# zhaozijie2022/LocoTouch

Hardware: AMD Instinct MI355X
Metric: env-steps/sec (whole node), TransportTeacher 4096 envs/GPU (higher is better)
Workload: dtype f32

## Files before the change

locotouch_amd/csrc/lt_wgrad.hip:

```cpp
#include <hip/hip_runtime.h>
#include <stdint.h>

#include "lt_env.h"
#include "lt_host_check.h"
#include "lt_internal.h"

namespace {

typedef float f32x4 __attribute__((ext_vector_type(4)));
typedef float f32x2 __attribute__((ext_vector_type(2)));
typedef _Float16 f16x8 __attribute__((ext_vector_type(8)));
typedef _Float16 f16x2 __attribute__((ext_vector_type(2)));

constexpr int TA = 4, TB = 4;
constexpr float LO_SCALE = 64.f;

template <int U>
__device__ __forceinline__ void split8(const f32x4 (&v)[8], float scale, f16x8& hi, f16x8& lo) {
#pragma unroll
  for (int p = 0; p < 4; ++p) {
    f32x2 x;
    x[0] = v[2 * p][U] * scale; x[1] = v[2 * p + 1][U] * scale;
    const f16x2 h = __builtin_convertvector(x, f16x2);
    const f32x2 d = (x - __builtin_convertvector(h, f32x2)) * LO_SCALE;
    const f16x2 l = __builtin_convertvector(d, f16x2);
    hi[2 * p] = h[0]; hi[2 * p + 1] = h[1];
    lo[2 * p] = l[0]; lo[2 * p + 1] = l[1];
  }
}

template <int U>
__device__ __forceinline__ void unpack8(const f32x4 (&v)[8], f16x8& hi, f16x8& lo) {
  typedef unsigned u32x4 __attribute__((ext_vector_type(4)));
  u32x4 h, l;
#pragma unroll
  for (int p = 0; p < 4; ++p) {
    const unsigned w0 = __float_as_uint(v[2 * p][U]), w1 = __float_as_uint(v[2 * p + 1][U]);
    h[p] = __builtin_amdgcn_perm(w1, w0, 0x05040100u);
    l[p] = __builtin_amdgcn_perm(w1, w0, 0x07060302u);
  }
  hi = __builtin_bit_cast(f16x8, h);
  lo = __builtin_bit_cast(f16x8, l);
}

struct WgradArgs {
  const float* dz;
  const float* x;
  long long M;
  int N, K;
  int tiles_n, tiles_k, splits;
  const float* amax;
  int nblk_amax;
  float* slabs;
  int dz_split;
  const float* dz_scale;
  int x_split;
  float* db;
};

constexpr int WG_WAVES = 4;
template <bool AS, bool XS>
__global__ __launch_bounds__(64 * WG_WAVES, 2) void lt_wgrad_kernel(const WgradArgs a) {
  __shared__ f32x4 s_tile[WG_WAVES - 1][TA * TB + 1][64];
  const int lane = threadIdx.x & 63;
  const int wave = __builtin_amdgcn_readfirstlane((int)threadIdx.x >> 6);
  const int i = lane & 15, g = lane >> 4;
  const int tiles = a.tiles_n * a.tiles_k;
  const int per_xcd = (int)gridDim.x >> 3;
  const int item = ((int)blockIdx.x & 7) * per_xcd + ((int)blockIdx.x >> 3);
  if (item >= tiles * a.splits) return;
  const int split = item / tiles, tile = item - split * tiles;
  const int tn = tile / a.tiles_k, tk = tile - tn * a.tiles_k;
  const int n0 = tn * 16 * TA, k0 = tk * 16 * TB;
  const long long steps = (a.M + 31) / 32;
  const long long b0 = steps * split / a.splits, b1 = steps * (split + 1) / a.splits;
  const long long s0 = b0 + (b1 - b0) * wave / WG_WAVES, s1 = b0 + (b1 - b0) * (wave + 1) / WG_WAVES;
  float scale = 1.f;
  if (AS) {
    scale = *a.dz_scale;
  } else if (a.amax) {
    float m = 0.f;
    for (int b = lane; b < a.nblk_amax; b += 64) m = fmaxf(m, a.amax[b]);
#pragma unroll
    for (int off = 32; off > 0; off >>= 1) m = fmaxf(m, __shfl_xor(m, off, 64));
    const int e = (int)((__float_as_uint(m) >> 23) & 0xFF) - 127;
    int se = 7 - e;
    se = se > 100 ? 100 : (se < -100 ? -100 : se);
    scale = __uint_as_float((unsigned)(127 + se) << 23);
  }
  f32x4 acc[TA][TB];
#pragma unroll
  for (int p = 0; p < TA; ++p)
#pragma unroll
    for (int q = 0; q < TB; ++q) acc[p][q] = f32x4{0.f, 0.f, 0.f, 0.f};
  f32x4 va[8], vb[8];
  const int ca = min(n0 + 4 * i, a.N - 4), cb = min(k0 + 4 * i, a.K - 4);
  const unsigned row_a = (unsigned)a.N * 4u, row_b = (unsigned)a.K * 4u;
  const unsigned last_a = (unsigned)(a.M - 1) * row_a + (unsigned)ca * 4u, last_b = (unsigned)(a.M - 1) * row_b + (unsigned)cb * 4u;
  unsigned off_a = ((unsigned)s0 * 32u + (unsigned)g) * row_a + (unsigned)ca * 4u, off_b = ((unsigned)s0 * 32u + (unsigned)g) * row_b + (unsigned)cb * 4u;
  auto issue = [&](long long) __attribute__((always_inline)) {
#pragma unroll
    for (int t = 0; t < 8; ++t) {
      va[t] = *(const f32x4*)((const char*)a.dz + min(off_a + (unsigned)(4 * t) * row_a, last_a));
      vb[t] = *(const f32x4*)((const char*)a.x + min(off_b + (unsigned)(4 * t) * row_b, last_b));
    }
    off_a += 32u * row_a;
    off_b += 32u * row_b;
  };
  const bool colsum = a.db != nullptr && tk == 0;
  f32x4 cs = f32x4{0.f, 0.f, 0.f, 0.f};
  if (s0 < s1) issue(s0);
  for (long long s = s0; s < s1; ++s) {
    if ((s + 1) * 32 > a.M) {
#pragma unroll
      for (int t = 0; t < 8; ++t) if (s * 32 + 4 * t + g >= a.M) va[t] = f32x4{0.f, 0.f, 0.f, 0.f};
    }
    if (colsum) {
      if (AS) {
#pragma unroll
        for (int t = 0; t < 8; ++t)
#pragma unroll
          for (int u = 0; u < 4; ++u) {
            const unsigned w = __float_as_uint(va[t][u]);
            cs[u] += (float)__builtin_bit_cast(_Float16, (unsigned short)(w & 0xFFFFu)) + (float)__builtin_bit_cast(_Float16, (unsigned short)(w >> 16)) * (1.f / LO_SCALE);
          }
      } else {
#pragma unroll
        for (int t = 0; t < 8; ++t) cs += va[t];
      }
    }
    f16x8 ah[TA], al[TA], bh[TB], bl[TB];
    if (AS) {
      unpack8<0>(va, ah[0], al[0]); unpack8<1>(va, ah[1], al[1]); unpack8<2>(va, ah[2], al[2]); unpack8<3>(va, ah[3], al[3]);
    } else {
      split8<0>(va, scale, ah[0], al[0]); split8<1>(va, scale, ah[1], al[1]); split8<2>(va, scale, ah[2], al[2]); split8<3>(va, scale, ah[3], al[3]);
    }
    if (XS) {
      unpack8<0>(vb, bh[0], bl[0]); unpack8<1>(vb, bh[1], bl[1]); unpack8<2>(vb, bh[2], bl[2]); unpack8<3>(vb, bh[3], bl[3]);
    } else {
      split8<0>(vb, 1.f, bh[0], bl[0]); split8<1>(vb, 1.f, bh[1], bl[1]); split8<2>(vb, 1.f, bh[2], bl[2]); split8<3>(vb, 1.f, bh[3], bl[3]);
    }
    if (s + 1 < s1) issue(s + 1);
#pragma unroll
    for (int p = 0; p < TA; ++p) {
      const f16x8 a64 = ah[p] * (_Float16)LO_SCALE;
#pragma unroll
      for (int q = 0; q < TB; ++q) {
        acc[p][q] = __builtin_amdgcn_mfma_f32_16x16x32_f16(a64, bh[q], acc[p][q], 0, 0, 0);
        acc[p][q] = __builtin_amdgcn_mfma_f32_16x16x32_f16(ah[p], bl[q], acc[p][q], 0, 0, 0);
        acc[p][q] = __builtin_amdgcn_mfma_f32_16x16x32_f16(al[p], bh[q], acc[p][q], 0, 0, 0);
      }
    }
  }
  if (wave > 0) {
#pragma unroll
    for (int p = 0; p < TA; ++p)
#pragma unroll
      for (int q = 0; q < TB; ++q) s_tile[wave - 1][p * TB + q][lane] = acc[p][q];
    s_tile[wave - 1][TA * TB][lane] = cs;
  }
  __syncthreads();
  if (wave > 0) return;
#pragma unroll
  for (int w = 0; w < WG_WAVES - 1; ++w) {
#pragma unroll
    for (int p = 0; p < TA; ++p)
#pragma unroll
      for (int q = 0; q < TB; ++q) acc[p][q] += s_tile[w][p * TB + q][lane];
    cs += s_tile[w][TA * TB][lane];
  }
  if (colsum) {
#pragma unroll
    for (int u = 0; u < 4; ++u) {
      cs[u] += __shfl_xor(cs[u], 16, 64);
      cs[u] += __shfl_xor(cs[u], 32, 64);
    }
    if (AS) cs *= 1.f / scale;
    if (g == 0 && n0 + 4 * i < a.N) *(f32x4*)(a.db + (long long)split * a.N + n0 + 4 * i) = cs;
  }
  const float inv = 1.f / (scale * LO_SCALE);
  float* const out = a.slabs + (long long)split * a.N * a.K;
  const int k = k0 + 4 * i;
#pragma unroll
  for (int p = 0; p < TA; ++p)
#pragma unroll
    for (int r = 0; r < 4; ++r) {
      const int n = n0 + 4 * (4 * g + r) + p;
      if (n < a.N && k < a.K) {
        f32x4 o;
#pragma unroll
        for (int q = 0; q < TB; ++q) o[q] = acc[p][q][r] * inv;
        *(f32x4*)(out + (long long)n * a.K + k) = o;
      }
    }
}

int pick_splits(long long M, int tiles) {
  const long long steps = (M + 31) / 32;
  long long s = 512 / tiles;
  if (s > steps / 8) s = steps / 8;
  return (int)(s < 1 ? 1 : s);
}

}

extern "C" int lt_wgrad_splits(int64_t M, int N, int K) {
  const int tiles = ((N + 16 * TA - 1) / (16 * TA)) * ((K + 16 * TB - 1) / (16 * TB));
  return pick_splits((long long)M, tiles);
}

extern "C" int64_t lt_wgrad_ws_floats(int64_t M, int N, int K) { return (int64_t)lt_wgrad_splits(M, N, K) * N * K; }

extern "C" int lt_wgrad(const float* dz, int dz_split, const float* dz_scale, const float* x, int x_split, int64_t M, int N, int K, const float* amax_blocks,
                        int nblk_amax, float* slabs, float* db_slabs, void* stream) {
  if (!dz || !x || !slabs || M < 1 || N < 4 || K < 4 || (N & 3) || (K & 3) || (amax_blocks && nblk_amax < 1) || (long long)M * (N > K ? N : K) * 4 >= (1ll << 32))
    return einval("lt_wgrad: invalid argument (N and K multiples of 4, each operand below 4 GiB)");
  WgradArgs a;
  a.dz = dz; a.x = x; a.M = M; a.N = N; a.K = K;
  a.amax = amax_blocks; a.nblk_amax = amax_blocks ? nblk_amax : 0;
  a.slabs = slabs; a.db = db_slabs; a.x_split = x_split != 0; a.dz_split = dz_split != 0; a.dz_scale = dz_scale;
  if (a.dz_split && !dz_scale) return einval("lt_wgrad: a split dz needs its scale");
  a.tiles_n = (N + 16 * TA - 1) / (16 * TA);
  a.tiles_k = (K + 16 * TB - 1) / (16 * TB);
  a.splits = pick_splits((long long)M, a.tiles_n * a.tiles_k);
  const dim3 grid((unsigned)((a.tiles_n * a.tiles_k * a.splits + 7) / 8 * 8));
  if (a.dz_split && a.x_split) hipLaunchKernelGGL((lt_wgrad_kernel<true, true>), grid, dim3(64 * WG_WAVES), 0, (hipStream_t)stream, a);
  else if (a.x_split) hipLaunchKernelGGL((lt_wgrad_kernel<false, true>), grid, dim3(64 * WG_WAVES), 0, (hipStream_t)stream, a);
  else if (a.dz_split) hipLaunchKernelGGL((lt_wgrad_kernel<true, false>), grid, dim3(64 * WG_WAVES), 0, (hipStream_t)stream, a);
  else hipLaunchKernelGGL((lt_wgrad_kernel<false, false>), grid, dim3(64 * WG_WAVES), 0, (hipStream_t)stream, a);
  return launch_status();
}

namespace {
__global__ __launch_bounds__(256) void lt_split_rows_kernel(const float* __restrict__ x, unsigned* __restrict__ out, long long n4) {
  typedef unsigned u32x4 __attribute__((ext_vector_type(4)));
  const long long i = (long long)blockIdx.x * 256 + threadIdx.x;
  if (i >= n4) return;
  const f32x4 v = ((const f32x4*)x)[i];
  u32x4 o;
#pragma unroll
  for (int k = 0; k < 4; ++k) {
    const float c = __builtin_amdgcn_fmed3f(v[k], -(float)LT_MLP_INPUT_CLAMP, (float)LT_MLP_INPUT_CLAMP);
    const _Float16 h = (_Float16)c;
    const _Float16 l = (_Float16)((c - (float)h) * LO_SCALE);
    o[k] = (unsigned)__builtin_bit_cast(unsigned short, h) | ((unsigned)__builtin_bit_cast(unsigned short, l) << 16);
  }
  ((u32x4*)out)[i] = o;
}
}

extern "C" int lt_split_rows(const float* x, void* out, int64_t count, void* stream) {
  if (!x || !out || count < 4 || (count & 3)) return einval("lt_split_rows: invalid argument (count a multiple of 4)");
  hipLaunchKernelGGL(lt_split_rows_kernel, dim3((unsigned)((count / 4 + 255) / 256)), dim3(256), 0, (hipStream_t)stream, x, (unsigned*)out, (long long)(count / 4));
  return launch_status();
}
```

Measured before the change: 68.32 million.

## Share split operand fragments across waves via LDS in wgrad kernel

Restructures the weight-gradient kernel so each workgroup covers a 2x2 block of 64x64 tiles with eight waves in two quads. In each quad, a wave loads and splits only one operand (dz or x) and exchanges the fp16 hi/lo fragments with a neighbour through double-buffered LDS. This removes the duplicate global loads and split work that separate tiles did before. It adds an LDS barrier per step, dynamic LDS allocation, and different split/grid sizing (MAX_WG 256, steps/4).

```diff
diff --git a/locotouch_amd/csrc/lt_wgrad.hip b/locotouch_amd/csrc/lt_wgrad.hip
--- a/locotouch_amd/csrc/lt_wgrad.hip
+++ b/locotouch_amd/csrc/lt_wgrad.hip
@@ -48,7 +48,7 @@
   const float* x;
   long long M;
   int N, K;
-  int tiles_n, tiles_k, splits;
+  int blocks_n, blocks_k, splits;
   const float* amax;
   int nblk_amax;
   float* slabs;
@@ -58,23 +58,119 @@
   float* db;
 };
 
-constexpr int WG_WAVES = 4;
+template <bool SPLIT>
+__device__ __forceinline__ void fragments(const f32x4 (&v)[8], float scale, f16x8 (&hi)[4], f16x8 (&lo)[4]) {
+  if (SPLIT) {
+    unpack8<0>(v, hi[0], lo[0]); unpack8<1>(v, hi[1], lo[1]); unpack8<2>(v, hi[2], lo[2]); unpack8<3>(v, hi[3], lo[3]);
+  } else {
+    split8<0>(v, scale, hi[0], lo[0]); split8<1>(v, scale, hi[1], lo[1]); split8<2>(v, scale, hi[2], lo[2]); split8<3>(v, scale, hi[3], lo[3]);
+  }
+}
+
+__device__ __forceinline__ void mma_tile(f32x4 (&acc)[TA][TB], const f16x8 (&ah)[TA], const f16x8 (&al)[TA], const f16x8 (&bh)[TB], const f16x8 (&bl)[TB]) {
+#pragma unroll
+  for (int p = 0; p < TA; ++p) {
+    const f16x8 a64 = ah[p] * (_Float16)LO_SCALE;
+#pragma unroll
+    for (int q = 0; q < TB; ++q) {
+      acc[p][q] = __builtin_amdgcn_mfma_f32_16x16x32_f16(a64, bh[q], acc[p][q], 0, 0, 0);
+      acc[p][q] = __builtin_amdgcn_mfma_f32_16x16x32_f16(ah[p], bl[q], acc[p][q], 0, 0, 0);
+      acc[p][q] = __builtin_amdgcn_mfma_f32_16x16x32_f16(al[p], bh[q], acc[p][q], 0, 0, 0);
+    }
+  }
+}
+
+__device__ __forceinline__ void lds_barrier() { asm volatile("s_waitcnt lgkmcnt(0)\n\ts_barrier" ::: "memory"); }
+
+constexpr int QUAD = 4;
+constexpr int WG_WAVES = 2 * QUAD;
+constexpr int PF = 1;
+constexpr int PANEL = 8 * 64;
+constexpr int LDS_BYTES = 2 * 2 * QUAD * PANEL * 16;
+constexpr int MAX_WG = 256;
+
+template <bool OWN_A, bool SPLIT, bool AS, bool COLSUM>
+__device__ __forceinline__ void sweep(const char* base, int M, int width, int col0, int g, int h0, int m_end, int trips, float scale, f16x8* post,
+                                      const f16x8* take, f32x4 (&acc)[TA][TB], f32x4& cs) {
+  const int col = min(col0, width - 4);
+  const unsigned row = (unsigned)width * 4u;
+  const unsigned last = (unsigned)(M - 1) * row + (unsigned)col * 4u;
+  unsigned off = ((unsigned)h0 * 32u + (unsigned)g) * row + (unsigned)col * 4u;
+  auto issue = [&](f32x4 (&v)[8]) __attribute__((always_inline)) {
+#pragma unroll
+    for (int t = 0; t < 8; ++t) v[t] = *(const f32x4*)(base + min(off + (unsigned)(4 * t) * row, last));
+    off += 32u * row;
+  };
+  f32x4 raw[PF][8];
+#pragma unroll
+  for (int j = 0; j < PF; ++j) {
+    issue(raw[j]);
+    __builtin_amdgcn_sched_barrier(0);
+  }
+  for (int it = 0; it < trips; it += PF) {
+#pragma unroll
+    for (int j = 0; j < PF; ++j) {
+      f32x4 (&v)[8] = raw[j];
+      const int left = m_end - (h0 + it + j) * 32 - g;
+#pragma unroll
+      for (int t = 0; t < 8; ++t)
+#pragma unroll
+        for (int u = 0; u < 4; ++u) v[t][u] = 4 * t < left ? v[t][u] : 0.f;
+      if (COLSUM) {
+        if (AS) {
+#pragma unroll
+          for (int t = 0; t < 8; ++t)
+#pragma unroll
+            for (int u = 0; u < 4; ++u) {
+              const unsigned w = __float_as_uint(v[t][u]);
+              cs[u] += (float)__builtin_bit_cast(_Float16, (unsigned short)(w & 0xFFFFu)) + (float)__builtin_bit_cast(_Float16, (unsigned short)(w >> 16)) * (1.f / LO_SCALE);
+            }
+        } else {
+#pragma unroll
+          for (int t = 0; t < 8; ++t) cs += v[t];
+        }
+      }
+      f16x8 oh[4], ol[4], fh[4], fl[4];
+      fragments<SPLIT>(v, scale, oh, ol);
+      const int buf = ((it + j) & 1) * QUAD * PANEL;
+#pragma unroll
+      for (int u = 0; u < 4; ++u) {
+        post[buf + (2 * u) * 64] = oh[u];
+        post[buf + (2 * u + 1) * 64] = ol[u];
+      }
+      issue(v);
+      lds_barrier();
+#pragma unroll
+      for (int u = 0; u < 4; ++u) {
+        fh[u] = take[buf + (2 * u) * 64];
+        fl[u] = take[buf + (2 * u + 1) * 64];
+      }
+      if (OWN_A) mma_tile(acc, oh, ol, fh, fl);
+      else mma_tile(acc, fh, fl, oh, ol);
+    }
+  }
+}
+
 template <bool AS, bool XS>
-__global__ __launch_bounds__(64 * WG_WAVES, 2) void lt_wgrad_kernel(const WgradArgs a) {
-  __shared__ f32x4 s_tile[WG_WAVES - 1][TA * TB + 1][64];
+__global__ __launch_bounds__(64 * WG_WAVES) void lt_wgrad_kernel(const WgradArgs a) {
+  extern __shared__ __attribute__((aligned(16))) unsigned char s_lds[];
   const int lane = threadIdx.x & 63;
   const int wave = __builtin_amdgcn_readfirstlane((int)threadIdx.x >> 6);
+  const int quad = wave >> 2, wq = wave & 3;
   const int i = lane & 15, g = lane >> 4;
-  const int tiles = a.tiles_n * a.tiles_k;
+  const int blocks = a.blocks_n * a.blocks_k;
   const int per_xcd = (int)gridDim.x >> 3;
   const int item = ((int)blockIdx.x & 7) * per_xcd + ((int)blockIdx.x >> 3);
-  if (item >= tiles * a.splits) return;
-  const int split = item / tiles, tile = item - split * tiles;
-  const int tn = tile / a.tiles_k, tk = tile - tn * a.tiles_k;
-  const int n0 = tn * 16 * TA, k0 = tk * 16 * TB;
-  const long long steps = (a.M + 31) / 32;
-  const long long b0 = steps * split / a.splits, b1 = steps * (split + 1) / a.splits;
-  const long long s0 = b0 + (b1 - b0) * wave / WG_WAVES, s1 = b0 + (b1 - b0) * (wave + 1) / WG_WAVES;
+  if (item >= blocks * a.splits) return;
+  const int split = item / blocks, block = item - split * blocks;
+  const int bn = block / a.blocks_k, bk = block - bn * a.blocks_k;
+  const bool own_a = !(wq & 1);
+  const int n0 = bn * 32 * TA + (((wq + 1) >> 1) & 1) * 16 * TA, k0 = bk * 32 * TB + (wq >> 1) * 16 * TB;
+  const int steps = (int)((a.M + 31) / 32);
+  const int b0 = (int)((long long)steps * split / a.splits), b1 = (int)((long long)steps * (split + 1) / a.splits);
+  const int h0 = b0 + (b1 - b0) * quad / 2, h1 = b0 + (b1 - b0) * (quad + 1) / 2;
+  const int trips = ((b1 - b0 + 1) / 2 + PF - 1) / PF * PF;
+  const int m_end = min((int)a.M, h1 * 32);
   float scale = 1.f;
   if (AS) {
     scale = *a.dz_scale;
@@ -93,82 +189,30 @@
   for (int p = 0; p < TA; ++p)
 #pragma unroll
     for (int q = 0; q < TB; ++q) acc[p][q] = f32x4{0.f, 0.f, 0.f, 0.f};
-  f32x4 va[8], vb[8];
-  const int ca = min(n0 + 4 * i, a.N - 4), cb = min(k0 + 4 * i, a.K - 4);
-  const unsigned row_a = (unsigned)a.N * 4u, row_b = (unsigned)a.K * 4u;
-  const unsigned last_a = (unsigned)(a.M - 1) * row_a + (unsigned)ca * 4u, last_b = (unsigned)(a.M - 1) * row_b + (unsigned)cb * 4u;
-  unsigned off_a = ((unsigned)s0 * 32u + (unsigned)g) * row_a + (unsigned)ca * 4u, off_b = ((unsigned)s0 * 32u + (unsigned)g) * row_b + (unsigned)cb * 4u;
-  auto issue = [&](long long) __attribute__((always_inline)) {
-#pragma unroll
-    for (int t = 0; t < 8; ++t) {
-      va[t] = *(const f32x4*)((const char*)a.dz + min(off_a + (unsigned)(4 * t) * row_a, last_a));
-      vb[t] = *(const f32x4*)((const char*)a.x + min(off_b + (unsigned)(4 * t) * row_b, last_b));
-    }
-    off_a += 32u * row_a;
-    off_b += 32u * row_b;
-  };
-  const bool colsum = a.db != nullptr && tk == 0;
   f32x4 cs = f32x4{0.f, 0.f, 0.f, 0.f};
-  if (s0 < s1) issue(s0);
-  for (long long s = s0; s < s1; ++s) {
-    if ((s + 1) * 32 > a.M) {
-#pragma unroll
-      for (int t = 0; t < 8; ++t) if (s * 32 + 4 * t + g >= a.M) va[t] = f32x4{0.f, 0.f, 0.f, 0.f};
-    }
-    if (colsum) {
-      if (AS) {
-#pragma unroll
-        for (int t = 0; t < 8; ++t)
-#pragma unroll
-          for (int u = 0; u < 4; ++u) {
-            const unsigned w = __float_as_uint(va[t][u]);
-            cs[u] += (float)__builtin_bit_cast(_Float16, (unsigned short)(w & 0xFFFFu)) + (float)__builtin_bit_cast(_Float16, (unsigned short)(w >> 16)) * (1.f / LO_SCALE);
-          }
-      } else {
-#pragma unroll
-        for (int t = 0; t < 8; ++t) cs += va[t];
-      }
-    }
-    f16x8 ah[TA], al[TA], bh[TB], bl[TB];
-    if (AS) {
-      unpack8<0>(va, ah[0], al[0]); unpack8<1>(va, ah[1], al[1]); unpack8<2>(va, ah[2], al[2]); unpack8<3>(va, ah[3], al[3]);
-    } else {
-      split8<0>(va, scale, ah[0], al[0]); split8<1>(va, scale, ah[1], al[1]); split8<2>(va, scale, ah[2], al[2]); split8<3>(va, scale, ah[3], al[3]);
-    }
-    if (XS) {
-      unpack8<0>(vb, bh[0], bl[0]); unpack8<1>(vb, bh[1], bl[1]); unpack8<2>(vb, bh[2], bl[2]); unpack8<3>(vb, bh[3], bl[3]);
-    } else {
-      split8<0>(vb, 1.f, bh[0], bl[0]); split8<1>(vb, 1.f, bh[1], bl[1]); split8<2>(vb, 1.f, bh[2], bl[2]); split8<3>(vb, 1.f, bh[3], bl[3]);
-    }
-    if (s + 1 < s1) issue(s + 1);
-#pragma unroll
-    for (int p = 0; p < TA; ++p) {
-      const f16x8 a64 = ah[p] * (_Float16)LO_SCALE;
-#pragma unroll
-      for (int q = 0; q < TB; ++q) {
-        acc[p][q] = __builtin_amdgcn_mfma_f32_16x16x32_f16(a64, bh[q], acc[p][q], 0, 0, 0);
-        acc[p][q] = __builtin_amdgcn_mfma_f32_16x16x32_f16(ah[p], bl[q], acc[p][q], 0, 0, 0);
-        acc[p][q] = __builtin_amdgcn_mfma_f32_16x16x32_f16(al[p], bh[q], acc[p][q], 0, 0, 0);
-      }
-    }
-  }
-  if (wave > 0) {
+  f16x8* const mail = (f16x8*)s_lds + quad * 2 * QUAD * PANEL + lane;
+  const bool colsum = a.db != nullptr && own_a && bk == 0;
+  f16x8* const post = mail + wq * PANEL;
+  const f16x8* const take = mail + ((wq + 1) & 3) * PANEL;
+  if (colsum) sweep<true, AS, AS, true>((const char*)a.dz, (int)a.M, a.N, n0 + 4 * i, g, h0, m_end, trips, scale, post, take, acc, cs);
+  else if (own_a) sweep<true, AS, AS, false>((const char*)a.dz, (int)a.M, a.N, n0 + 4 * i, g, h0, m_end, trips, scale, post, take, acc, cs);
+  else sweep<false, XS, AS, false>((const char*)a.x, (int)a.M, a.K, k0 + 4 * i, g, h0, m_end, trips, 1.f, post, take, acc, cs);
+  lds_barrier();
+  f32x4* const hand = (f32x4*)s_lds + wq * (TA * TB + 1) * 64 + lane;
+  if (quad > 0) {
 #pragma unroll
     for (int p = 0; p < TA; ++p)
 #pragma unroll
-      for (int q = 0; q < TB; ++q) s_tile[wave - 1][p * TB + q][lane] = acc[p][q];
-    s_tile[wave - 1][TA * TB][lane] = cs;
+      for (int q = 0; q < TB; ++q) hand[(p * TB + q) * 64] = acc[p][q];
+    hand[TA * TB * 64] = cs;
   }
   __syncthreads();
-  if (wave > 0) return;
-#pragma unroll
-  for (int w = 0; w < WG_WAVES - 1; ++w) {
-#pragma unroll
-    for (int p = 0; p < TA; ++p)
-#pragma unroll
-      for (int q = 0; q < TB; ++q) acc[p][q] += s_tile[w][p * TB + q][lane];
-    cs += s_tile[w][TA * TB][lane];
-  }
+  if (quad > 0) return;
+#pragma unroll
+  for (int p = 0; p < TA; ++p)
+#pragma unroll
+    for (int q = 0; q < TB; ++q) acc[p][q] += hand[(p * TB + q) * 64];
+  cs += hand[TA * TB * 64];
   if (colsum) {
 #pragma unroll
     for (int u = 0; u < 4; ++u) {
@@ -195,19 +239,29 @@
     }
 }
 
-int pick_splits(long long M, int tiles) {
+int pick_splits(long long M, int blocks) {
   const long long steps = (M + 31) / 32;
-  long long s = 512 / tiles;
-  if (s > steps / 8) s = steps / 8;
+  long long s = MAX_WG / blocks;
+  if (s > steps / 4) s = steps / 4;
   return (int)(s < 1 ? 1 : s);
 }
 
-}
-
-extern "C" int lt_wgrad_splits(int64_t M, int N, int K) {
-  const int tiles = ((N + 16 * TA - 1) / (16 * TA)) * ((K + 16 * TB - 1) / (16 * TB));
-  return pick_splits((long long)M, tiles);
-}
+int blocks_of(int n) { return (n + 32 * TA - 1) / (32 * TA); }
+
+template <bool AS, bool XS>
+int launch(const WgradArgs& a, hipStream_t stream) {
+  if (const int e = lt_ensure_dynamic_lds((const void*)lt_wgrad_kernel<AS, XS>, LDS_BYTES)) {
+    lt_set_error(hipGetErrorString((hipError_t)e));
+    return LT_EHIP;
+  }
+  const dim3 grid((unsigned)((a.blocks_n * a.blocks_k * a.splits + 7) / 8 * 8));
+  hipLaunchKernelGGL((lt_wgrad_kernel<AS, XS>), grid, dim3(64 * WG_WAVES), (size_t)LDS_BYTES, stream, a);
+  return launch_status();
+}
+
+}
+
+extern "C" int lt_wgrad_splits(int64_t M, int N, int K) { return pick_splits((long long)M, blocks_of(N) * blocks_of(K)); }
 
 extern "C" int64_t lt_wgrad_ws_floats(int64_t M, int N, int K) { return (int64_t)lt_wgrad_splits(M, N, K) * N * K; }
 
@@ -220,15 +274,13 @@
   a.amax = amax_blocks; a.nblk_amax = amax_blocks ? nblk_amax : 0;
   a.slabs = slabs; a.db = db_slabs; a.x_split = x_split != 0; a.dz_split = dz_split != 0; a.dz_scale = dz_scale;
   if (a.dz_split && !dz_scale) return einval("lt_wgrad: a split dz needs its scale");
-  a.tiles_n = (N + 16 * TA - 1) / (16 * TA);
-  a.tiles_k = (K + 16 * TB - 1) / (16 * TB);
-  a.splits = pick_splits((long long)M, a.tiles_n * a.tiles_k);
-  const dim3 grid((unsigned)((a.tiles_n * a.tiles_k * a.splits + 7) / 8 * 8));
-  if (a.dz_split && a.x_split) hipLaunchKernelGGL((lt_wgrad_kernel<true, true>), grid, dim3(64 * WG_WAVES), 0, (hipStream_t)stream, a);
-  else if (a.x_split) hipLaunchKernelGGL((lt_wgrad_kernel<false, true>), grid, dim3(64 * WG_WAVES), 0, (hipStream_t)stream, a);
-  else if (a.dz_split) hipLaunchKernelGGL((lt_wgrad_kernel<true, false>), grid, dim3(64 * WG_WAVES), 0, (hipStream_t)stream, a);
-  else hipLaunchKernelGGL((lt_wgrad_kernel<false, false>), grid, dim3(64 * WG_WAVES), 0, (hipStream_t)stream, a);
-  return launch_status();
+  a.blocks_n = blocks_of(N);
+  a.blocks_k = blocks_of(K);
+  a.splits = pick_splits((long long)M, a.blocks_n * a.blocks_k);
+  if (a.dz_split && a.x_split) return launch<true, true>(a, (hipStream_t)stream);
+  if (a.x_split) return launch<false, true>(a, (hipStream_t)stream);
+  if (a.dz_split) return launch<true, false>(a, (hipStream_t)stream);
+  return launch<false, false>(a, (hipStream_t)stream);
 }
 
 namespace {
```

After: 68.40 million (median of 2 runs). About the same (+0.1%).
